# siisee11/PMDFC

Hardware: AMD Instinct MI355X
Metric: batched CCEH lookup+insert Mops/s (1/2/4/8 GPU) + % HBM random-access roofline (higher is better)
Workload: dtype u64; 1 GPU; config2: per GPU 64M unique uniform u64 keys (value=key), CCEH_hybrid(65536); 64 Insert batches of 1M then 64 Get batches of 1M (100% hit); index reset each step; the insert batches through InsertBatches (batch i+1 partitioned while batch i is applied), the Get batches through GetBatches (one launch over the 64 batches; per-op results as batch by batch); keys_per_gpu=67108864, batch=1048576, init_cap=65536, parallelism=hash-prefix shards x1

## Files before the change

pmdfc_amd/csrc/bucket.hip:

```cpp
#include <algorithm>
#include <cstdlib>
#include <cstddef>

#include "cceh_device.h"
#include "cceh_kernels.h"
#include "knobs.h"

namespace pmdfc {

constexpr int kPartThreads = 1024;
constexpr int kPartPer = (int)kPartTile / kPartThreads;

constexpr int kCW = (int)kChunkWave;
constexpr int kPer = kCW / 64;
constexpr int kBmLanes = 30;
constexpr int kRoundGuard = 64;

constexpr uint32_t kGetBit = 0x80000000u;
constexpr uint32_t kOpMask = (1u << 22) - 1;

__device__ __forceinline__ uint64_t sk_make(uint32_t seg, uint32_t op, uint32_t i, uint32_t home) {
  return ((uint64_t)seg << 39) | ((uint64_t)op << 17) | ((uint64_t)i << 8) | home;
}
__device__ __forceinline__ uint32_t sk_seg(uint64_t k) { return (uint32_t)(k >> 39); }
// ... 1314 lines not shown
      if (dmask[u] & F.unres[xc]) {
        blocked_any = true;
        continue;
      }
      const uint32_t v = F.opk[p], wo = (v & 0xFFu) * 4u, q0 = F.dst[xc];
      uint32_t occw = F.snap[p];
      bool park = false;
      for (uint32_t m = dmask[u]; m; m &= m - 1u) {
        const uint32_t rq = F.res[q0 + (uint32_t)__builtin_ctz(m)];
        const uint32_t ds = ((rq & (kSlots - 1)) - wo) & (kSlots - 1);
        park |= (rq & (kFrFull | kFrPark)) != 0;
        if ((rq & kFrClaim) && ds < kWindow) occw |= 1u << ds;
      }
      if (park) {
        nr[u] = kFrPark;
      } else if (~occw) {
        nr[u] = kFrClaim | ((wo + (uint32_t)__builtin_ctz(~occw)) & (kSlots - 1));
      } else {
        nr[u] = kFrFull;
        atomicMin(&F.bfull[xc], v >> 8);
      }
    }
    __builtin_amdgcn_wave_barrier();
#pragma unroll
    for (int u = 0; u < kLp; ++u) {
      if (!nr[u]) continue;
      const uint32_t p = (uint32_t)u * 64u + lane, xc = F.binp[p];
      F.res[p] = (uint16_t)nr[u];
      atomicAnd(&F.unres[xc], ~(1u << (p - F.dst[xc])));
      lres[u] = nr[u];
    }
    __builtin_amdgcn_wave_barrier();
    if (!__ballot(blocked_any)) break;
  }
  stamp(srow, kBsFcResolved, lane == 0);
  if (srow && lane == 0) srow[kBsFcRounds] = nrounds | ((uint64_t)ntot << 16);
}

template <bool UPS, uint32_t NL, uint32_t NB, class BinF>
__device__ __forceinline__ void fc_commit(const BucketArgs& a, uint32_t w, const FcScr<NL, NB>& F, const LaneOps& o,
                                          const bool (&pc)[kPer], const uint32_t (&st)[kPer], BinF bin,
                                          ulonglong2* wl_kv, uint32_t* wl_op, uint32_t* s_nsplit, uint32_t* s_nreq,
                                          uint32_t* s_need, WaveStat& c, const uint32_t* upd) {
  const uint32_t lbase = a.sbits + a.p1;
#pragma unroll
  for (int j = 0; j < kPer; ++j) {
    if (!o.pq[j]) continue;
    const uint32_t op = o.rop[j] & kOpMask, bf = F.bfull[bin(j)];
    const uint32_t r = st[j] & 0xFFFFu;
    const uint32_t seg = de_seg(o.e8[j]);
    if (op >= bf || (r & kFrPark)) {
      if (op == bf) {
        const uint32_t L = de_ld(o.e8[j]);
        const uint32_t ri = a.mode == 2 ? kSplitCap : atomicAdd(s_nreq, 1u);
        if (ri < kSplitCap) {
          a.req[(size_t)w * kSplitCap + ri] = make_uint2(seg | (L << 27), o.x8[j]);
          a.reqop[(size_t)w * kSplitCap + ri] = op;
          atomicMax(s_need, L + 1 - lbase);
        }
      }
      const uint32_t k = atomicAdd(s_nsplit, 1u);
      wl_kv[k] = make_ulonglong2(o.rk[j], o.rv[j]);
      wl_op[k] = o.rop[j];
      ++c.waited;
    } else if (r & kFrClaim) {
      const uint32_t sl = r & (kSlots - 1);
      a.pairs[(size_t)seg * kSlots + sl] = make_ulonglong2(o.rk[j], o.rv[j]);
      atomicOr(a.occ + (size_t)seg * 32u + (sl >> 5), 1u << (sl & 31u));
      c.lines += (((sl - o.home8[j] * 4u) & (kSlots - 1)) >> 2) + 1u;
    } else if (UPS && !pc[j]) {
      const uint32_t sl = upd[j];
      a.pairs[(size_t)seg * kSlots + sl] = make_ulonglong2(o.rk[j], o.rv[j]);
      a.st[op] = 11;
      c.lines += (((sl - o.home8[j] * 4u) & (kSlots - 1)) >> 2) + 1u;
    }
  }
}

template <uint32_t NL, uint32_t NB, bool UPS = false, class BinF>
__device__ __forceinline__ bool fast_claim(const BucketArgs& a, uint32_t w, uint32_t* sc,
                                           const uint64_t* s_key, ulonglong2* wl_kv, uint32_t* wl_op,
                                           uint32_t* s_nsplit, uint32_t* s_nreq, uint32_t* s_need,
                                           const LaneOps& o, BinF bin, WaveStat& c, uint64_t* srow,
                                           const uint32_t* upd = nullptr, const uint32_t* occw = nullptr) {
  const uint32_t lane = __lane_id() & 63u;
  const uint32_t full = a.ctl->full;
  const FcScr<NL, NB> F(sc);
  uint32_t *const hm = F.hm, *const dm = F.dm, *const cnt = F.cnt, *const dst = F.dst, *const bfull = F.bfull;
  bool pc[kPer];
#pragma unroll
  for (int j = 0; j < kPer; ++j) pc[j] = o.pq[j] && (!UPS || upd[j] == 0xFFFFu);
  uint32_t olo[kPer], ohi[kPer];
#pragma unroll
  for (int j = 0; j < kPer; ++j) {
    if (!pc[j]) continue;
    if constexpr (UPS) {
      olo[j] = occw[2 * j];
      ohi[j] = occw[2 * j + 1];
    } else {
      const uint32_t* og = a.occ + (size_t)de_seg(o.e8[j]) * 32u;
      const uint32_t wi = o.home8[j] >> 3;
      olo[j] = ld_u32_l2(og + wi);
      ohi[j] = ld_u32_l2(og + ((wi + 1u) & 31u));
    }
  }
#pragma unroll
  for (int t = 0; t < (int)(2 * NB * 8 / 64); ++t) hm[t * 64 + lane] = 0;
  if (lane < NB) {
    cnt[lane] = 0;
    bfull[lane] = 0xFFFFFFFFu;
  }
  __builtin_amdgcn_wave_barrier();
  uint32_t st[kPer];
#pragma unroll
  for (int j = 0; j < kPer; ++j)
    if (pc[j]) st[j] = atomicOr(&hm[bin(j) * 8u + (o.home8[j] >> 5)], 1u << (o.home8[j] & 31u));
#pragma unroll
  for (int j = 0; j < kPer; ++j)
    if (pc[j] && ((st[j] >> (o.home8[j] & 31u)) & 1u)) atomicOr(&dm[bin(j) * 8u + (o.home8[j] >> 5)], 1u << (o.home8[j] & 31u));
  __builtin_amdgcn_wave_barrier();
  stamp(srow, kBsBinned, lane == 0);
  if (srow && lane == 0) srow[kBsOrdered] = 0;
  constexpr uint32_t kDep = 1u << 24;
  uint64_t fk = 0;
  int fkj = -1;
#pragma unroll
  for (int j = 0; j < kPer; ++j) {
    st[j] = 0;
    if (!pc[j]) continue;
    const uint32_t h = o.home8[j], xc = bin(j), base = xc * 8u, l0 = (h - 7u) & 255u;
    const uint32_t wo = h * 4u;
    const uint32_t win = __builtin_amdgcn_alignbit(ohi[j], olo[j], wo & 31u);
    const uint32_t cl = ~win ? (uint32_t)__builtin_ctz(~win) >> 2 : 7u;
    const uint32_t w0 = hm[base + (l0 >> 5)], w1 = hm[base + (((l0 >> 5) + 1u) & 7u)];
    const uint32_t nb = __builtin_amdgcn_alignbit(w1, w0, l0 & 31u) & ((0x100u << cl) - 1u) & ~0x80u;
    const bool dup = (dm[base + (h >> 5)] >> (h & 31u)) & 1u;
    if (nb != 0 || dup) {
      const uint32_t r = atomicAdd(&cnt[xc], 1u);
      st[j] = kDep | (r << 16);
    } else if (~win) {
      st[j] = kFrClaim | ((wo + (uint32_t)__builtin_ctz(~win)) & (kSlots - 1));
    } else {
      st[j] = kFrFull;
      atomicMin(&bfull[xc], o.rop[j] & kOpMask);
      if (fkj < 0) {
        fk = ld_pair_l2(a.pairs + (size_t)de_seg(o.e8[j]) * kSlots + wo).x;
        fkj = j;
      }
    }
  }
  __builtin_amdgcn_wave_barrier();
  const uint32_t cb = lane < NB ? cnt[lane] : 0u;
  if (__ballot(cb > kDepMax)) return false;
  uint32_t ntot;
  const uint32_t ex = wave_excl_scan(cb, &ntot);
  if (lane < NB) dst[lane] = ex;
  uint32_t runs = 0;
  if (lane < NB) {
    uint32_t any = 0;
#pragma unroll
    for (int t = 0; t < 8; ++t) any |= hm[lane * 8u + t];
    runs = (uint32_t)__popcll(__ballot(any != 0));
  }
  __builtin_amdgcn_wave_barrier();
  stamp(srow, kBsBatchOrder, lane == 0);
#pragma unroll
  for (int j = 0; j < kPer; ++j) {
    if (!(st[j] & kDep)) continue;
    const uint32_t xc = bin(j), p = dst[xc] + ((st[j] >> 16) & 0xFFu);
    st[j] = kDep | (p << 16);
    F.opk[p] = ((o.rop[j] & kOpMask) << 8) | o.home8[j];
    F.snap[p] = __builtin_amdgcn_alignbit(ohi[j], olo[j], (o.home8[j] * 4u) & 31u);
    F.res[p] = 0;
    F.slot8[p] = (uint8_t)((uint32_t)j * 64u + lane);
    F.binp[p] = (uint8_t)xc;
  }
  if (lane < NB) F.unres[lane] = cb >= 32 ? 0xFFFFFFFFu : (1u << cb) - 1u;
  __builtin_amdgcn_wave_barrier();
  fc_resolve(F, ntot, srow);
#pragma unroll
  for (int j = 0; j < kPer; ++j)
    if (st[j] & kDep) st[j] |= F.res[(st[j] >> 16) & 0xFFu];
  bool fails = false;
#pragma unroll
  for (int j = 0; j < kPer; ++j) {
    if (!pc[j] || (o.rop[j] & kOpMask) != bfull[bin(j)]) continue;
    const uint32_t xc = bin(j), q0 = (st[j] & kDep) ? dst[xc] : 0u, n = (st[j] & kDep) ? cnt[xc] : 0u;
    if (fkj == j && hash64(fk) != hash64(o.rk[j])) {
      fails |= de_ld(o.e8[j]) + 1 > kMaxDepth || full;
      continue;
    }
    fails |= fc_full(a, full, o.e8[j], o.rk[j], o.home8[j] * 4u, F.res, F.slot8, s_key, q0, n) != kFrSplit;
  }
  if (__ballot(fails)) return false;
  stamp(srow, kBsRunsDone, lane == 0);
  fc_commit<UPS>(a, w, F, o, pc, st, bin, wl_kv, wl_op, s_nsplit, s_nreq, s_need, c, upd);
  if (lane == 0) c.runs += runs;
  stamp(srow, kBsWritten, lane == 0);
  return true;
}

__device__ __forceinline__ void clear_other_parity(const BucketArgs& a) {
  const uint32_t lane = __lane_id() & 63u, q = a.par ^ 1u;
  if (lane < 2 * kGShards) a.gsh[((size_t)q * kGShards + (lane % kGShards)) * kGStride + (lane / kGShards) * 16] = 0;
  if (lane == 2 * kGShards) a.ctl->nfin[q] = 0;
  if (lane == 2 * kGShards + 1) a.ctl->anyreq[q] = 0;
  if (lane == 2 * kGShards + 2) a.ctl->anydecl[q] = 0;
}


__device__ __forceinline__ void first_pass_clears(const BucketArgs& a, uint32_t w) {
  const uint32_t lane = __lane_id() & 63u;
  const uint32_t pb = w >> a.sbb, sub = w & ((1u << a.sbb) - 1);
  if (a.clear_next) {
    if (sub == 0 && lane < kPartSubs) a.cursor_next[(lane << (a.p1 - a.sbb)) + pb] = 0;
    if (w == 0 && lane == 0) *a.ovf_next = 0;
  }
  if (w == 0) clear_other_parity(a);
}

constexpr int kPre = 4;
static_assert(kPre * 64 == 32 * kPartSubs, "prefetch: 32 records per sub-region");
struct PreRecs {
  uint32_t op[kPre];
  uint64_t k[kPre], v[kPre];
};
__device__ __forceinline__ void prefetch_records(const BucketArgs& a, uint32_t pb, uint32_t half, PreRecs& pr) {
  const uint32_t lane = __lane_id() & 63u;
  const uint64_t rb0 = (uint64_t)pb * a.cap;
#pragma unroll
  for (int u = 0; u < kPre; ++u) {
    const uint32_t jj = (uint32_t)u * 64u + lane;
    const uint64_t j = rb0 + (uint64_t)(jj >> 5) * a.capx + min(half * 32u + (jj & 31u), a.capx - 1u);
    pr.op[u] = a.rop[j];
    const ulonglong2 kv = a.rkv[j];
    pr.k[u] = kv.x;
    pr.v[u] = kv.y;
  }
}
__device__ __forceinline__ bool pre_valid(const BucketArgs& a, const PreRecs& pr, int u, uint32_t half, uint32_t csub,
                                          uint32_t sub) {
  const uint32_t jj = (uint32_t)u * 64u + (__lane_id() & 63u);
  const uint32_t cs = (uint32_t)__shfl((int)csub, (int)(jj >> 5));
  return half * 32u + (jj & 31u) < cs && ((pr.op[u] >> 22) & ((1u << a.sbb) - 1)) == sub;
}
__device__ __forceinline__ uint32_t compact_prefetched(const BucketArgs& a, const PreRecs& pr, uint32_t half,
                                                       uint32_t csub, uint32_t sub, uint32_t m, ulonglong2* kv,
                                                       uint32_t* op, uint32_t cap) {
  const uint64_t lt = (1ULL << (__lane_id() & 63u)) - 1;
#pragma unroll
  for (int u = 0; u < kPre; ++u) {
    const bool match = pre_valid(a, pr, u, half, csub, sub);
    const uint64_t bal = __ballot(match);
    const uint32_t idx = m + (uint32_t)__popcll(bal & lt);
    if (match && idx < cap) {
      kv[idx] = make_ulonglong2(pr.k[u], pr.v[u]);
      op[idx] = pr.op[u];
    }
    m += (uint32_t)__popcll(bal);
  }
  return m;
}

__device__ __forceinline__ uint32_t sub_count_load(const BucketArgs& a, uint32_t pb) {
  const uint32_t lane = __lane_id() & 63u;
  return lane < kPartSubs ? min(a.cursor[(lane << (a.p1 - a.sbb)) + pb], a.capx) : 0u;
}
__device__ __forceinline__ uint32_t sub_count_max(uint32_t csub) {
  uint32_t cmax = csub;
#pragma unroll
  for (int o = 4; o > 0; o >>= 1) cmax = max(cmax, (uint32_t)__shfl_xor((int)cmax, o));
  return (uint32_t)__shfl((int)cmax, 0);
}

__device__ __forceinline__ void request_tail(const BucketArgs& a, uint32_t w, const uint32_t& nreq,
                                             const uint32_t& need, uint32_t db) {
  __builtin_amdgcn_wave_barrier();
  const uint32_t nr = min(nreq, kSplitCap);
  if (nr) request_splits(a, w, nr, need > db ? need : 0u);
}

__device__ __forceinline__ void publish_stats(const BucketArgs& a, uint32_t w, uint64_t wsv, WaveStat c) {
  const uint32_t lane = __lane_id() & 63u;
  for (int o = 32; o > 0; o >>= 1) {
    c.lines += (uint32_t)__shfl_down((int)c.lines, o);
    c.waited += (uint32_t)__shfl_down((int)c.waited, o);
  }
  const uint32_t s0 = (uint32_t)__shfl((int)c.lines, 0), s1 = (uint32_t)__shfl((int)c.waited, 0);
  const uint32_t s3 = (uint32_t)__shfl((int)c.loss, 0), s4 = (uint32_t)__shfl((int)c.runs, 0);
  const uint32_t add = lane == 0 ? s0 : lane == 1 ? s1 : lane == 2 ? c.splits : lane == 3 ? s3
                     : lane == 4 ? s4 : lane == 5 ? c.rounds : 0u;
  uint64_t* ws = a.wstat + (size_t)w * kWStat;
  if (lane < 6u && add) ws[lane] = wsv + add;
  if (lane == 3u && s3) atomicAdd(&a.ctl->loss_events, 1u);
  if (lane == 6u && (c.max_rounds || c.max_ld || c.grow)) {
    const uint64_t mr = max((uint32_t)(wsv & 0xFFFF), c.max_rounds);
    const uint64_t ml = max((uint32_t)((wsv >> 16) & 0xFF), c.max_ld);
    ws[6] = mr | (ml << 16) | (((wsv >> 32) + c.grow) << 32);
  }
  if (lane == 0 && c.bad) atomicOr(&a.ctl->err, 4u);
}



static_assert(kPre == kPer, "the prefetched records fill the chunk registers slot for slot");

struct ChunkRegs {
  uint64_t k[kPer], v[kPer];
  uint32_t op[kPer];
  bool ok[kPer];
};

struct RoundOps {
  bool pq[kPer];
  uint64_t kk[kPer];
  uint32_t ro[kPer];
  uint32_t e8[kPer], home8[kPer], x8[kPer];
};

__device__ __forceinline__ uint32_t chunk_slot(bool strided, int j) {
  const uint32_t lane = __lane_id() & 63u;
  return strided ? (uint32_t)j * 64u + lane : kPer * lane + (uint32_t)j;
}

struct LdsDir {
  bool on = false, written = false;
  uint32_t v0 = 0, v1 = 0;
};
__device__ __forceinline__ LdsDir lds_dir_load(const BucketArgs& a, uint32_t off, uint32_t db) {
  const uint32_t lane = __lane_id() & 63u;
  LdsDir d;
  d.on = (1u << db) <= kLdsDir;
  if (d.on) {
    if (lane < (1u << db)) d.v0 = ld_u32_l2(a.pool + off + lane);
    if (lane + 64u < (1u << db)) d.v1 = ld_u32_l2(a.pool + off + lane + 64u);
  }
  return d;
}

__device__ __forceinline__ void take_chunk(const ulonglong2* kv, const uint32_t* op, uint32_t m, ChunkRegs& r) {
#pragma unroll
  for (int j = 0; j < kPer; ++j) {
    const uint32_t i = (uint32_t)j * 64u + (__lane_id() & 63u);
    r.ok[j] = i < m;
    if (r.ok[j]) {
      const ulonglong2 p = kv[i];
      r.k[j] = p.x;
      r.v[j] = p.y;
      r.op[j] = op[i];
// ... 717 lines not shown
#pragma unroll
  for (int q = 0; q < kPer; ++q) {
    const uint32_t pv = q ? v[q - 1] : (lane ? prev_last : ~0u);
    const bool st = v[q] != ~0u && (pv == ~0u || (pv >> 8) != (v[q] >> 8));
    starts |= st ? 1u << q : 0u;
    s_rank[kPer * lane + q] = v[q];
  }
  uint32_t tot;
  const uint32_t rk0 = wave_excl_scan((uint32_t)__builtin_popcount(starts), &tot);
  if (lane == 0) s_sel[0] = ~0u;
  __builtin_amdgcn_wave_barrier();
  if (blockIdx.x >= tot) return;
  {
    uint32_t r = rk0;
#pragma unroll
    for (int q = 0; q < kPer; ++q)
      if ((starts >> q) & 1u) {
        if (r == blockIdx.x) {
          s_sel[0] = v[q] >> 8;
          s_sel[1] = kPer * lane + q;
        }
        ++r;
      }
  }
  __builtin_amdgcn_wave_barrier();
  const uint32_t w = s_sel[0], e0 = s_sel[1];
  uint32_t m = 0;
  for (uint32_t t0 = 0; e0 + t0 < kCW; t0 += 64) {
    const uint32_t t = t0 + lane;
    const uint32_t e = e0 + t < kCW ? s_rank[e0 + t] : ~0u;
    const bool mine = e != ~0u && (e >> 8) == w;
    const uint64_t bal = __ballot(mine);
    m += (uint32_t)__popcll(bal);
    if (mine) {
      const uint32_t i = e & 0xFFu;
      const bool ins = !ops || ops[i] == 1;
      S.kv[t] = make_ulonglong2(keys[i], ins ? vin[i] : 0ULL);
      S.op[t] = i | (ins ? 0u : kGetBit);
      if (ins && a.vout) a.vout[i] = 0;
    }
    if (bal != ~0ULL) break;
  }
  __builtin_amdgcn_wave_barrier();
  bucket_body<true, true, false>(a, w, S, m);
}

__device__ __forceinline__ bool tiny_batch(const BucketArgs& a, BucketLds<true, false>& S, uint32_t n, bool in,
                                           uint64_t key, bool ins, uint64_t val,
                                           const uint64_t* hdr_cache = nullptr) {
  const uint32_t lane = threadIdx.x & 63u;
  const uint64_t h = hash64(key);
  bool live = false;
  if (in) {
    const uint8_t bad = reserved_key(key) ? 3 : wrong_shard(h, a.sbits, a.shard) ? 8 : 0;
    if (bad) {
      a.st[lane] = bad;
      if (a.vout) a.vout[lane] = 0;
    }
    live = !bad;
  }
  const uint32_t w = live ? bucket_of(h, a.sbits, a.p1) : 0u;
  uint32_t e = 0;
  if (live) {
    const uint64_t hd = hdr_cache ? hdr_cache[w] : a.hdr[w];
    e = ld_u32_l2(a.pool + hdr_off(hd) + sub_index(h, a.sbits, a.p1, hdr_db(hd)));
  }
  const uint32_t seg = de_seg(e);
  const uint64_t lv = __ballot(live);
  bool shared = false;
  for (uint64_t m = lv; m; m &= m - 1) {
    const int j = __builtin_ctzll(m);
    const uint32_t sj = (uint32_t)__shfl((int)seg, j);
    shared |= (uint32_t)j != lane && sj == seg;
  }
  bool general = live && (shared || (ins && a.upsert));
  if (live && !general) {
    ulonglong2* sp = a.pairs + (size_t)seg * kSlots;
    if (!ins) {
      uint64_t v = 0;
      const uint8_t st = lane_probe(sp, key, h, &v);
      a.vout[lane] = v;
      a.st[lane] = st;
    } else {
      const uint32_t wi0 = (uint32_t)(h & 0xFF) * 4u, wi = wi0 >> 5, wn = (wi + 1u) & 31u;
      uint32_t* og = a.occ + (size_t)seg * 32u;
      const uint32_t lo = ld_u32_l2(og + wi), hi = ld_u32_l2(og + wn);
      const int pos = window_first_free(lo, hi, wi0);
      if (pos < 0) {
        general = true;
      } else {
        sp[pos] = make_ulonglong2(key, val);
        const uint32_t pw = (uint32_t)pos >> 5;
        og[pw] = (pw == wi ? lo : hi) | (1u << ((uint32_t)pos & 31u));
        a.st[lane] = 2;
        if (a.vout) a.vout[lane] = 0;
      }
    }
  }
  const bool any_general = __ballot(general) != 0;
  for (uint64_t gm = __ballot(general); gm;) {
    const uint32_t wb = (uint32_t)__shfl((int)w, __builtin_ctzll(gm));
    const uint64_t mine = __ballot(general && w == wb);
    if (general && w == wb) {
      const uint32_t t = (uint32_t)__popcll(mine & ((1ULL << lane) - 1));
      S.kv[t] = make_ulonglong2(key, val);
      S.op[t] = lane | (ins ? 0u : kGetBit);
      if (ins && a.vout) a.vout[lane] = 0;
    }
    __builtin_amdgcn_s_waitcnt(0);
    __builtin_amdgcn_wave_barrier();
    bucket_body<true, true, false>(a, wb, S, (uint32_t)__popcll(mine));
    __builtin_amdgcn_wave_barrier();
    gm &= ~mine;
  }
  return any_general;
}

__global__ __launch_bounds__(64, 1) void k_mixed_tiny(BucketArgs a, const uint8_t* __restrict__ ops,
                                                      const uint64_t* __restrict__ keys,
                                                      const uint64_t* __restrict__ vin) {
  __shared__ BucketLds<true, false> S;
  const uint32_t lane = threadIdx.x, n = (uint32_t)a.n;
  const bool in = lane < n;
  const uint64_t key = in ? keys[lane] : kInvalid;
  const bool ins = in && (!ops || ops[lane] == 1);
  const uint64_t val = ins ? vin[lane] : 0ULL;
  tiny_batch(a, S, n, in, key, ins, val);
}

__device__ __forceinline__ uint32_t sys_ld32(const uint32_t* p) {
  return __hip_atomic_load(p, __ATOMIC_RELAXED, __HIP_MEMORY_SCOPE_SYSTEM);
}
__device__ __forceinline__ uint64_t sys_ld64(const uint64_t* p) {
  return __hip_atomic_load(p, __ATOMIC_RELAXED, __HIP_MEMORY_SCOPE_SYSTEM);
}
__device__ __forceinline__ void sys_st32(uint32_t* p, uint32_t v) {
  __hip_atomic_store(p, v, __ATOMIC_RELAXED, __HIP_MEMORY_SCOPE_SYSTEM);
}
__device__ __forceinline__ void sys_st64(uint64_t* p, uint64_t v) {
  __hip_atomic_store(p, v, __ATOMIC_RELAXED, __HIP_MEMORY_SCOPE_SYSTEM);
}

__global__ __launch_bounds__(64, 1) void k_serve(ServeArgs sa) {
  __shared__ BucketLds<true, false> S;
  const uint32_t lane = threadIdx.x;
  const uint64_t mask = sa.ring_size - 1;
  if (sa.nwaves > 1) {
    sa.req += (size_t)blockIdx.x * sa.ring_size;
    sa.resp += (size_t)blockIdx.x * sa.ring_size;
    sa.ctl += blockIdx.x;
    sa.head0 = sys_ld64(&sa.ctl->head);
  }
  uint64_t head = sa.head0, chunks = 0, reloads = 0;
  uint64_t hb = sys_ld64(&sa.ctl->heartbeat);
  uint64_t t_hb = (uint64_t)wall_clock64(), t_last = t_hb;
  bool idle_set = false;
  uint64_t tp[5] = {0, 0, 0, 0, 0};
  const uint64_t t_start = t_hb;
  const auto put_prof = [&] {
    const uint64_t life = (uint64_t)wall_clock64() - t_start;
    if (lane < 6)
      sys_st64(&sa.ctl->prof[lane],
               lane == 0 ? tp[0] : lane == 1 ? tp[1] : lane == 2 ? tp[2] : lane == 3 ? tp[3] : lane == 4 ? tp[4] : life);
    if (lane == 6) sys_st64(&sa.ctl->head, head);
    if (lane == 7) sys_st64(&sa.ctl->chunks, chunks);
    if (lane == 8) sys_st64(&sa.ctl->reloads, reloads);
  };
  __shared__ uint8_t s_st[64];
  __shared__ uint64_t s_vout[64];
// ... 146 lines not shown
      if (!ok) a.ctl->full = 1;
    }
    if (!ok) {
      if (gs + nr <= a.max_segments && (!team || wv == 0)) {
        retire_segment(a.pairs, a.occ, a.ldep, seg0 + k);
        if (lane == 0) atomicAdd(&a.ctl->dead, 1u);
      }
      continue;
    }
    bool b = false;
    uint64_t* stp = a.stamps && k < kSplitStamps ? a.stamps + (size_t)k * 8 : nullptr;
    stamp(stp, kSsStart, lane == 0 && (!team || wv == 0));
    const uint32_t trig = a.drops ? a.reqop[(size_t)w * kSplitCap + i] : 0u;
    const uint32_t ps = el.x & ((1u << 27) - 1), pl = el.x >> 27;
    if (team) {
      loss += split_team<4>(a.pairs, a.occ, a.ldep, ps, seg0 + k, pl, &s_scr[0][0], &b, stp, a.drops, &a.ctl->drop_n,
                            trig, wv);
    } else {
      uint32_t so = wv * kSplitScratch;
      __asm__ volatile("" : "+v"(so));
      loss += wave_split(a.pairs, a.occ, a.ldep, ps, seg0 + k, pl, &s_scr[0][0] + so, &b, stp, a.drops,
                         &a.ctl->drop_n, trig);
    }
    bad |= b;
  }
  if (lane == 0 && (!team || wv == 0)) {
    if (loss) {
      atomicAdd(reinterpret_cast<unsigned long long*>(&a.ctl->split_loss), (unsigned long long)loss);
      atomicAdd(&a.ctl->loss_events, 1u);
    }
    if (bad) atomicOr(&a.ctl->err, 4u);
  }
}

static SplitArgs split_args(const BucketArgs& a, uint64_t* stamps, uint32_t team_max) {
  SplitArgs p;
  p.par = a.par;
  p.pfix = a.pfix;
  p.stamps = stamps;
  p.gsh = a.gsh;
  p.gsplit = a.gsplit;
  p.gcap = a.gcap;
  p.act = a.act;
  p.gbase = a.gbase;
  p.ngrant = a.ngrant;
  p.newoff = a.newoff;
  p.need = a.need;
  p.max_segments = a.max_segments;
  p.pool_cap = a.pool_cap;
  p.pairs = a.pairs;
  p.occ = a.occ;
  p.ldep = a.ldep;
  p.ctl = a.ctl;
  p.reqop = a.reqop;
  p.drops = a.drops;
  p.team_max = team_max;
  return p;
}

template <bool WIDE>
struct FastCfg {
  static constexpr int FP = WIDE ? 2 : 3;
  static constexpr uint32_t FC = 64u * (uint32_t)FP;
  static constexpr uint32_t NB = WIDE ? 64u : kFastBins;
  static constexpr uint32_t MaxDb = WIDE ? 7u : 5u;
};

template <bool WIDE>
struct FastLds {
  using C = FastCfg<WIDE>;
  union {
    uint32_t sc[FcLayout<C::FC, C::NB>::Words];
    struct {
      ulonglong2 kv[C::FC];
      uint32_t op[C::FC];
    } stage;
  };
  uint32_t seen[4];
  uint32_t nsplit, nreq, need;
};

constexpr uint32_t kCpWaves = 1u << kCpSbb;
constexpr uint32_t kCpPre = 192;
struct CpLds {
  union {
    FastLds<false> w[kCpWaves];
    struct {
      ulonglong2 kv[kPartSubs * kCpPre];
      uint32_t op[kPartSubs * kCpPre];
      uint16_t idx[kCpWaves][FastCfg<false>::FC];
    } st;
  };
  uint32_t csub[kPartSubs];
};
static_assert(sizeof(CpLds) <= 40 * 1024, "4 workgroups of 8 waves per CU");

__device__ __forceinline__ bool dense_bins(uint32_t* seen, const bool (&pq)[kPer], uint32_t (&bn)[kPer], uint32_t nb) {
  __builtin_amdgcn_wave_barrier();
#pragma unroll
  for (int j = 0; j < kPer; ++j)
    if (pq[j]) atomicOr(&seen[bn[j] >> 5], 1u << (bn[j] & 31u));
  __builtin_amdgcn_wave_barrier();
  const uint32_t s0 = seen[0], s1 = seen[1], s2 = seen[2], s3 = seen[3];
  if (__builtin_popcount(s0) + __builtin_popcount(s1) + __builtin_popcount(s2) + __builtin_popcount(s3) > (int)nb)
    return false;
#pragma unroll
  for (int j = 0; j < kPer; ++j) {
    const uint32_t x = bn[j], q = x >> 5, below = (1u << (x & 31u)) - 1u;
    uint32_t r = __builtin_popcount((q == 0 ? s0 : q == 1 ? s1 : q == 2 ? s2 : s3) & below);
    r += q > 0 ? __builtin_popcount(s0) : 0;
    r += q > 1 ? __builtin_popcount(s1) : 0;
    r += q > 2 ? __builtin_popcount(s2) : 0;
    bn[j] = r;
  }
  return true;
}

__device__ __forceinline__ bool upsert_probe(const BucketArgs& a, const bool (&pq)[kPer], const uint64_t (&rk)[kPer],
                                             const uint32_t (&e8)[kPer], const uint32_t (&home8)[kPer],
                                             uint32_t (&upd)[kPer], uint32_t (&occw)[2 * kPer]) {
  const uint32_t lane = __lane_id() & 63u;
  uint32_t hv[4];
#pragma unroll
  for (int q = 0; q < 4; ++q) hv[q] = q < kPer && pq[q] ? (uint32_t)hash64(rk[q]) : 0xFFFFFFFFu;
  wave_sort32<4>(hv, 256);
  bool dup = false;
#pragma unroll
  for (int q = 0; q < 3; ++q) dup |= hv[q] != 0xFFFFFFFFu && hv[q] == hv[q + 1];
  const uint32_t nx = (uint32_t)__shfl_down((int)hv[0], 1);
  dup |= lane < 63u && hv[3] != 0xFFFFFFFFu && hv[3] == nx;
  if (__ballot(dup)) return false;
  uint32_t nl[kPer];
#pragma unroll
  for (int j = 0; j < kPer; ++j) {
    upd[j] = 0xFFFFu;
    occw[2 * j] = occw[2 * j + 1] = 0;
    if (!pq[j]) continue;
    const uint32_t* og = a.occ + (size_t)de_seg(e8[j]) * 32u;
    const uint32_t wi = home8[j] >> 3;
    occw[2 * j] = ld_u32_l2(og + wi);
    occw[2 * j + 1] = ld_u32_l2(og + ((wi + 1u) & 31u));
  }
#pragma unroll
  for (int j = 0; j < kPer; ++j) {
    const uint32_t win = __builtin_amdgcn_alignbit(occw[2 * j + 1], occw[2 * j], (home8[j] * 4u) & 31u);
    const uint32_t ff = ~win ? (uint32_t)__builtin_ctz(~win) : 32u;
    nl[j] = pq[j] ? (ff + 3u) >> 2 : 0u;
  }
  for (uint32_t t = 0;; ++t) {
    bool more = false;
#pragma unroll
    for (int j = 0; j < kPer; ++j) more |= t < nl[j] && upd[j] == 0xFFFFu;
    if (!__ballot(more)) break;
    uint64_t kq[kPer][4];
#pragma unroll
    for (int j = 0; j < kPer; ++j) {
      if (t >= nl[j] || upd[j] != 0xFFFFu) continue;
      const ulonglong2* ln = a.pairs + (size_t)de_seg(e8[j]) * kSlots + ((home8[j] + t) & 255u) * 4u;
#pragma unroll
      for (int q = 0; q < 4; ++q) kq[j][q] = reinterpret_cast<const uint64_t*>(ln + q)[0];
    }
#pragma unroll
    for (int j = 0; j < kPer; ++j) {
      if (t >= nl[j] || upd[j] != 0xFFFFu) continue;
#pragma unroll
      for (int q = 3; q >= 0; --q)
        if (kq[j][q] == rk[j]) upd[j] = ((home8[j] + t) * 4u + (uint32_t)q) & (kSlots - 1);
    }
  }
  return true;
}

template <bool WIDE, bool UPS = false, bool CP = false>
__device__ __forceinline__ uint32_t apply_fast(const BucketArgs& a, FastLds<WIDE>& S, uint32_t w,
                                               CpLds* cpl = nullptr) {
  using C = FastCfg<WIDE>;
  static_assert(!CP || (!WIDE && !UPS), "the coarse-partition pass is the lean insert-only one");
  const uint32_t lane = threadIdx.x & 63u;
  const uint32_t pb = w >> a.sbb, sub = w & ((1u << a.sbb) - 1);
  uint64_t* const srow = bucket_stamp_row(a, w);
  stamp(srow, kBsStart, lane == 0);
  first_pass_clears(a, w);
  PreRecs pr;
  constexpr int kCpLd = (int)(kPartSubs * kCpPre / (64 * kCpWaves));
  static_assert(kCpLd <= kPre, "the staging loads use the prefetch registers");
  if constexpr (CP) {
    const uint64_t rb0 = (uint64_t)pb * a.cap;
#pragma unroll
    for (int u = 0; u < kCpLd; ++u) {
      const uint32_t t = (uint32_t)u * 64u * kCpWaves + threadIdx.x;
      const uint64_t j = rb0 + (uint64_t)(t / kCpPre) * a.capx + min(t % kCpPre, a.capx - 1u);
      pr.op[u] = a.rop[j];
      const ulonglong2 kv = a.rkv[j];
      pr.k[u] = kv.x;
      pr.v[u] = kv.y;
    }
  } else {
    prefetch_records(a, pb, 0, pr);
  }
  const uint32_t csub = sub_count_load(a, pb);
  const uint64_t wsv = lane < 7u ? a.wstat[(size_t)w * kWStat + lane] : 0ULL;
  const uint32_t* fslot = a.pool + (size_t)w * kFixedSlot;
  const uint32_t spec0 = (a.pfix && (WIDE || lane < 32u)) ? ld_u32_l2(fslot + lane) : 0u;
  const uint32_t spec1 = (WIDE && a.pfix) ? ld_u32_l2(fslot + 64u + lane) : 0u;
  const uint64_t hd = a.hdr[w];
  const uint32_t off = hdr_off(hd), db = hdr_db(hd);
  const uint32_t novf = *a.ovf;
  const bool fixed = a.pfix && off == w * kFixedSlot && db <= kFixedBits;
  uint32_t dv0, dv1 = 0u;
  if (fixed) {
    dv0 = lane < (1u << db) ? spec0 : 0u;
    dv1 = lane + 64u < (1u << db) ? spec1 : 0u;
  } else {
    dv0 = (db <= C::MaxDb && lane < (1u << db)) ? ld_u32_l2(a.pool + off + lane) : 0u;
    if (WIDE) dv1 = (db <= C::MaxDb && lane + 64u < (1u << db)) ? ld_u32_l2(a.pool + off + 64u + lane) : 0u;
  }
  const uint32_t cmax = sub_count_max(csub);
  bool pq[kPer];
  uint64_t rk[kPer], rv[kPer];
  uint32_t rop[kPer];
  if constexpr (CP) {
#pragma unroll
    for (int u = 0; u < kCpLd; ++u) {
      const uint32_t t = (uint32_t)u * 64u * kCpWaves + threadIdx.x;
      cpl->st.op[t] = pr.op[u];
      cpl->st.kv[t] = make_ulonglong2(pr.k[u], pr.v[u]);
    }
    __syncthreads();
    uint32_t dec = (db > C::MaxDb || novf != 0) ? 2u : cmax > kCpPre ? 2u : 0u;
    uint32_t m = 0;
    if (!dec) {
      const uint64_t lt = (1ULL << lane) - 1;
      const uint32_t v = w & (kCpWaves - 1);
      uint16_t* my = cpl->st.idx[v];
#pragma unroll 4
      for (uint32_t c = 0; c < kPartSubs * kCpPre / 64; ++c) {
        const uint32_t t = c * 64u + lane;
        const uint32_t cs = (uint32_t)__shfl((int)csub, (int)(t / kCpPre));
        const uint32_t r = cpl->st.op[t];
        const bool match = t % kCpPre < cs && ((r >> 22) & (kCpWaves - 1)) == v;
        const uint64_t bal = __ballot(match);
        const uint32_t idx = m + (uint32_t)__popcll(bal & lt);
        if (match && idx < C::FC) my[idx] = (uint16_t)t;
        m += (uint32_t)__popcll(bal);
      }
      if (m > C::FC) dec = 1u;
      __builtin_amdgcn_wave_barrier();
#pragma unroll
      for (int j = 0; j < kPer; ++j) {
        const uint32_t i = (uint32_t)j * 64u + lane;
        pq[j] = !dec && j < C::FP && i < m;
        rk[j] = rv[j] = 0;
        rop[j] = 0;
        if (pq[j]) {
          const uint32_t t = my[i];
          const ulonglong2 kv = cpl->st.kv[t];
          rk[j] = kv.x;
          rv[j] = kv.y;
          rop[j] = cpl->st.op[t];
        }
      }
    }
    __syncthreads();
    if (dec) return dec;
  } else {
    if (db > C::MaxDb || novf != 0) return 2u;
    if (cmax > C::FC) return 1u;
    uint32_t m = 0;
    for (uint32_t half = 0; half * 32u < cmax; ++half) {
      if (half) prefetch_records(a, pb, half, pr);
      m = compact_prefetched(a, pr, half, csub, sub, m, S.stage.kv, S.stage.op, C::FC);
    }
    if (m > C::FC) return 1u;
    __builtin_amdgcn_wave_barrier();
#pragma unroll
    for (int j = 0; j < kPer; ++j) {
      const uint32_t i = (uint32_t)j * 64u + lane;
      pq[j] = j < C::FP && i < m;
      rk[j] = rv[j] = 0;
      rop[j] = 0;
      if (pq[j]) {
        const ulonglong2 kv = S.stage.kv[i];
        rk[j] = kv.x;
        rv[j] = kv.y;
        rop[j] = S.stage.op[i];
      }
    }
    __builtin_amdgcn_wave_barrier();
  }
  if (lane == 0) {
    S.nsplit = 0;
    S.nreq = 0;
    S.need = db;
  }
  if (WIDE && lane < 4) S.seen[lane] = 0;
  uint32_t e8[kPer], home8[kPer], x8[kPer], bn[WIDE ? kPer : 1];
  (void)bn;
#pragma unroll
  for (int j = 0; j < kPer; ++j) {
    home8[j] = x8[j] = 0;
    if (pq[j]) {
      const uint64_t h = hash64(rk[j]);
      home8[j] = (uint32_t)(h & 0xFF);
      x8[j] = sub_index(h, a.sbits, a.p1, db);
    }
    const uint32_t lo = (uint32_t)__shfl((int)dv0, (int)(x8[j] & 63u));
    if (WIDE) {
      const uint32_t hi = (uint32_t)__shfl((int)dv1, (int)(x8[j] & 63u));
      e8[j] = x8[j] < 64u ? lo : hi;
    } else {
      e8[j] = lo;
    }
  }
  const auto first_sub = [&](int j) -> uint32_t { return first_sub_index(a, db, x8[j], e8[j]); };
  if constexpr (WIDE) {
#pragma unroll
    for (int j = 0; j < kPer; ++j) bn[j] = pq[j] ? first_sub(j) : 0u;
    if (!dense_bins(S.seen, pq, bn, C::NB)) return 1u;
  }
  uint32_t upd[UPS ? kPer : 1], occw[UPS ? 2 * kPer : 1];
  if constexpr (UPS) {
    if (!upsert_probe(a, pq, rk, e8, home8, upd, occw)) return 1u;
  }
  stamp(srow, kBsLoaded, lane == 0);
  WaveStat c;
  const auto bin = [&](int j) -> uint32_t {
    if constexpr (WIDE) return bn[j];
    else return first_sub(j);
  };
  if (!fast_claim<C::FC, C::NB, UPS>(a, w, S.sc, nullptr, a.wl_kv + (size_t)w * kCW, a.wl_op + (size_t)w * kCW,
                                     &S.nsplit, &S.nreq, &S.need, LaneOps{rk, rv, rop, pq, e8, home8, x8}, bin, c, srow,
                                     UPS ? upd : nullptr, UPS ? occw : nullptr))
    return 1u;
  if (lane == 0) a.wl_n[w] = S.nsplit;
  request_tail(a, w, S.nreq, S.need, db);
  c.rounds = c.max_rounds = 1;
  publish_stats(a, w, wsv, c);
  stamp(srow, kBsEnd, lane == 0);
  return 0u;
}

__device__ __forceinline__ void declined(const BucketArgs& a, uint32_t w) {
  a.fbl[w] |= 1u;
  a.ctl->anydecl[a.par] = 1u;
}

__global__ __launch_bounds__(64, 8) void k_apply_fast(BucketArgs a) {
  if (gated_off(a)) return;
  __shared__ FastLds<false> S;
  if (apply_fast<false>(a, S, blockIdx.x) != 0 && threadIdx.x == 0) declined(a, blockIdx.x);
}

#ifndef PMDFC_CP_WPE
#define PMDFC_CP_WPE 8
#endif
__global__ __launch_bounds__(64 * kCpWaves) __attribute__((amdgpu_waves_per_eu(PMDFC_CP_WPE, 8))) void k_apply_fast_cp(
    BucketArgs a) {
  if (gated_off(a)) return;
  __shared__ CpLds L;
  const uint32_t v = (uint32_t)__builtin_amdgcn_readfirstlane((int)(threadIdx.x >> 6)), w = (blockIdx.x << kCpSbb) | v;
  if (apply_fast<false, false, true>(a, L.w[v], w, &L) != 0 && (threadIdx.x & 63u) == 0) declined(a, w);
}

__global__ __launch_bounds__(64, 6) void k_apply_wide(BucketArgs a) {
  if (gated_off(a)) return;
  __shared__ FastLds<true> S;
  if (apply_fast<true>(a, S, blockIdx.x) != 0 && threadIdx.x == 0) declined(a, blockIdx.x);
}

template <bool WIDE>
__global__ __launch_bounds__(64, 5) void k_apply_fast_ups(BucketArgs a) {
  __shared__ FastLds<WIDE> S;
  if (apply_fast<WIDE, true>(a, S, blockIdx.x) != 0 && threadIdx.x == 0) declined(a, blockIdx.x);
}

__global__ __launch_bounds__(64, 2) void k_apply_fb(BucketArgs a) {
  if (gated_off(a)) return;
  const uint32_t w = blockIdx.x, f = a.fbl[w];
  if (!(f & 1u)) return;
  __shared__ BucketLds<false, true> S;
  bucket_body<false, false, true>(a, w, S);
  if (threadIdx.x == 0) a.fbl[w] = f + 1u;
}


#ifndef PMDFC_PARKED_GRID
#define PMDFC_PARKED_GRID 3072
#endif
#ifndef PMDFC_FINAL_GRID
#define PMDFC_FINAL_GRID 256
#endif
constexpr uint32_t kParkedGrid = PMDFC_PARKED_GRID;
constexpr uint32_t kFinalGrid = PMDFC_FINAL_GRID;
#ifndef PMDFC_MIXED_SMALL_GRID
#define PMDFC_MIXED_SMALL_GRID 256
#endif
constexpr uint32_t kMixedSmallGrid = PMDFC_MIXED_SMALL_GRID;
#ifndef PMDFC_PARKED_GRID_RAMP
#define PMDFC_PARKED_GRID_RAMP 4096
#endif
#ifndef PMDFC_FINAL_GRID_RAMP
#define PMDFC_FINAL_GRID_RAMP 1024
#endif
constexpr uint32_t kParkedGridRamp = PMDFC_PARKED_GRID_RAMP;
constexpr uint32_t kFinalGridRamp = PMDFC_FINAL_GRID_RAMP;

uint32_t part_blocks(uint64_t n) { return (uint32_t)((n + kPartTile - 1) / kPartTile); }

void launch_part(const PartArgs& a, hipStream_t s) {
  if (!a.n) return;
  hipLaunchKernelGGL(k_part, dim3(part_blocks(a.n)), dim3(kPartThreads), 0, s, a);
}

void launch_apply(const BucketLaunch& L, uint32_t mode, hipStream_t s) {
  if (!L.a.n) return;
// ... 89 lines not shown
```

pmdfc_amd/csrc/cceh_device.h:

```cpp
#pragma once
#include <hip/hip_runtime.h>
#include <stdint.h>

namespace pmdfc {

constexpr uint32_t kSlots = 1024;
constexpr uint32_t kWindow = 32;
constexpr uint32_t kLines = 8;
constexpr uint32_t kMaxDepth = 30;
constexpr uint64_t kInvalid = ~0ULL;
constexpr uint64_t kSentinel = ~0ULL - 1;
constexpr uint8_t kStPending = 0xFF;
constexpr uint8_t kStLinked = 0xFE;
constexpr uint8_t kStJoin = 0xFD;
constexpr uint32_t kJoinReps = 8;
constexpr uint32_t kJoinBits = 1u << 20;
constexpr uint64_t kJoinWords = (uint64_t)kJoinBits / 32 * kJoinReps;
__host__ __device__ __forceinline__ uint64_t iset_slot(uint64_t h, uint64_t mask) {
  return (h ^ (h >> 29) ^ (h >> 47)) & mask;
}

__host__ __device__ __forceinline__ uint64_t hash64(uint64_t key) {
  const uint64_t mul = 0xc6a4a7935bd1e995ULL;
  uint64_t h = 0xc70697ULL ^ (8ULL * mul);
// ... 7 lines not shown

__host__ __device__ __forceinline__ uint32_t murmur2_u64(uint64_t key, uint32_t seed) {
  const uint32_t m = 0x5bd1e995u;
  uint32_t h = seed ^ 8u;
  uint32_t k = (uint32_t)key;
  k *= m; k ^= k >> 24; k *= m;
  h *= m; h ^= k;
  k = (uint32_t)(key >> 32);
  k *= m; k ^= k >> 24; k *= m;
  h *= m; h ^= k;
  h ^= h >> 13; h *= m; h ^= h >> 15;
  return h;
}

__host__ __device__ __forceinline__ uint64_t splitmix64(uint64_t x) {
  uint64_t z = x + 0x9E3779B97F4A7C15ULL;
  z = (z ^ (z >> 30)) * 0xBF58476D1CE4E5B9ULL;
  z = (z ^ (z >> 27)) * 0x94D049BB133111EBULL;
  return z ^ (z >> 31);
}

__host__ __device__ __forceinline__ bool reserved_key(uint64_t k) {
  return k >= kSentinel;
}

constexpr uint32_t kSegBits = 26;
constexpr uint32_t kSegMask = (1u << kSegBits) - 1;
constexpr uint64_t kMaxSegments = 1ULL << 25;
__host__ __device__ __forceinline__ uint32_t de_seg(uint32_t e) { return e & kSegMask; }
__host__ __device__ __forceinline__ uint32_t de_ld(uint32_t e) { return e >> kSegBits; }
__host__ __device__ __forceinline__ uint32_t de_make(uint32_t seg, uint32_t ld) {
  return seg | (ld << kSegBits);
}

struct Geo {
  const uint64_t* hdr;
  const uint32_t* pool;
  uint32_t p1;
  uint32_t sbits;
  uint32_t shard;
  const uint32_t* flat;
  const uint32_t* flat_bits;
};
constexpr uint32_t kFlatMaxBits = 20;

__host__ __device__ __forceinline__ uint32_t hdr_off(uint64_t hd) { return (uint32_t)hd; }
__host__ __device__ __forceinline__ uint32_t hdr_db(uint64_t hd) { return (uint32_t)(hd >> 32) & 0xFFu; }
__host__ __device__ __forceinline__ uint64_t hdr_make(uint32_t off, uint32_t db) {
  return (uint64_t)off | ((uint64_t)db << 32);
}

__device__ __forceinline__ uint32_t bucket_of(uint64_t h, uint32_t sbits, uint32_t p1) {
  return p1 ? (uint32_t)((h << sbits) >> (64 - p1)) : 0u;
}
__device__ __forceinline__ uint32_t sub_index(uint64_t h, uint32_t sbits, uint32_t p1, uint32_t db) {
  return db ? (uint32_t)((h << (sbits + p1)) >> (64 - db)) : 0u;
}

__device__ __forceinline__ uint32_t dir_entry(const Geo& g, uint64_t h) {
  if (g.flat) {
    const uint32_t fb = *g.flat_bits;
    if (fb <= kFlatMaxBits) return g.flat[fb ? (uint32_t)((h << g.sbits) >> (64 - fb)) : 0u];
  }
  const uint64_t hd = g.hdr[bucket_of(h, g.sbits, g.p1)];
  return g.pool[hdr_off(hd) + sub_index(h, g.sbits, g.p1, hdr_db(hd))];
}

__device__ __forceinline__ bool wrong_shard(uint64_t h, uint32_t sbits, uint32_t shard) {
  return sbits != 0 && (uint32_t)(h >> (64 - sbits)) != shard;
}

typedef unsigned long long u64x2_t __attribute__((ext_vector_type(2)));
typedef unsigned int u32x4_t __attribute__((ext_vector_type(4)));
__device__ __forceinline__ ulonglong2 ld_pair_l2(const ulonglong2* p) {
  const u64x2_t v = __builtin_nontemporal_load(reinterpret_cast<const u64x2_t*>(p));
  return make_ulonglong2(v.x, v.y);
}
__device__ __forceinline__ uint4 ld_u4_l2(const uint32_t* p) {
  const u32x4_t v = __builtin_nontemporal_load(reinterpret_cast<const u32x4_t*>(p));
  return make_uint4(v.x, v.y, v.z, v.w);
}
__device__ __forceinline__ uint32_t ld_u32_l2(const uint32_t* p) {
  return __hip_atomic_load(p, __ATOMIC_RELAXED, __HIP_MEMORY_SCOPE_AGENT);
}

__device__ __forceinline__ int window_first_free(uint32_t lo, uint32_t hi, uint32_t w) {
  uint64_t win = (((uint64_t)hi << 32) | lo) >> (w & 31);
  uint32_t fr = ~(uint32_t)win;
  if (fr == 0) return -1;
  return (int)((w + (uint32_t)__builtin_ctz(fr)) & (kSlots - 1));
}

__device__ __forceinline__ uint64_t shfl64(uint64_t v, int src) {
  int lo = __shfl((int)(uint32_t)v, src);
  int hi = __shfl((int)(uint32_t)(v >> 32), src);
  return ((uint64_t)(uint32_t)hi << 32) | (uint32_t)lo;
}

__device__ __forceinline__ uint8_t quad_probe(const ulonglong2* __restrict__ seg, uint64_t key,
                                              uint64_t h, uint32_t q, uint64_t* val,
                                              uint32_t* lines) {
  const uint32_t line0 = (uint32_t)(h & 0xFF);
  const uint32_t qbase = (__lane_id() & 63u) & ~3u;
  for (uint32_t t = 0; t < kLines;) {
    const uint32_t ln = (line0 + t) & 255u;
    const bool two = !(ln & 1u) && t + 1 < kLines;
    const ulonglong2 pa = seg[ln * 4u + q];
    const ulonglong2 pb = two ? seg[ln * 4u + 4u + q] : pa;
#pragma unroll
    for (uint32_t k = 0; k < 2; ++k) {
      if (k == 1 && !two) break;
      const ulonglong2 p = k ? pb : pa;
      const uint32_t mn = (uint32_t)(__ballot(p.x == key) >> qbase) & 0xFu;
      const uint32_t en = (uint32_t)(__ballot(p.x == kInvalid) >> qbase) & 0xFu;
      if (mn) {
        *val = shfl64(p.y, (int)(qbase + (uint32_t)__builtin_ctz(mn)));
        *lines = t + k + 1;
        return 1;
      }
      if (en) {
        *lines = t + k + 1;
        return 0;
      }
    }
    t += two ? 2u : 1u;
  }
  *lines = kLines;
  return 0;
}

__device__ __forceinline__ uint8_t quad_probe_once(const ulonglong2* __restrict__ seg, uint64_t key,
                                                   uint64_t h, uint32_t q, uint64_t* val) {
  const uint32_t line0 = (uint32_t)(h & 0xFF);
  const uint32_t qbase = (__lane_id() & 63u) & ~3u;
  uint32_t copies = 0;
  for (uint32_t t = 0; t < kLines;) {
    const uint32_t ln = (line0 + t) & 255u;
    const bool two = !(ln & 1u) && t + 1 < kLines;
    const ulonglong2 pa = seg[ln * 4u + q];
    const ulonglong2 pb = two ? seg[ln * 4u + 4u + q] : pa;
    bool stop = false;
#pragma unroll
    for (uint32_t k = 0; k < 2; ++k) {
      if (k == 1 && !two) break;
      const ulonglong2 p = k ? pb : pa;
      const uint32_t mn = (uint32_t)(__ballot(p.x == key) >> qbase) & 0xFu;
      const uint32_t en = (uint32_t)(__ballot(p.x == kInvalid) >> qbase) & 0xFu;
      if (mn && copies == 0) *val = shfl64(p.y, (int)(qbase + (uint32_t)__builtin_ctz(mn)));
      copies += (uint32_t)__builtin_popcount(mn);
      if (en || copies > 1) {
        stop = true;
        break;
      }
    }
    if (stop) break;
    t += two ? 2u : 1u;
  }
  return copies == 0 ? 0 : copies == 1 ? 1 : 2;
}

__device__ __forceinline__ uint8_t lane_probe(const ulonglong2* __restrict__ seg, uint64_t key,
                                              uint64_t h, uint64_t* val) {
  const uint32_t line0 = (uint32_t)(h & 0xFF);
  for (uint32_t t = 0; t < kLines; t += 2) {
    ulonglong2 ln[8];
#pragma unroll
// ... 139 lines not shown
```

Measured before the change: 13520 Mops/s.

## Split compaction staging loads into lean first stage and gated second stage

Refactors occupancy-window loads behind a WinLd helper. An optional 64-bit atomic load is added but left off by default. In the CP compaction path, the staging loads are split into a 128-record first stage and a 64-record second stage. The second stage is skipped when a sub-region's count does not reach it, and the header, overflow and count loads are issued early so they overlap the record loads. The compaction scan now walks each sub-region only up to its count, which is meant to avoid useless loads and LDS reads in exchange for more complex indexing and extra readlane work.

```diff
diff --git a/pmdfc_amd/csrc/bucket.hip b/pmdfc_amd/csrc/bucket.hip
--- a/pmdfc_amd/csrc/bucket.hip
+++ b/pmdfc_amd/csrc/bucket.hip
@@ -1420,7 +1420,7 @@
                                            const uint64_t* s_key, ulonglong2* wl_kv, uint32_t* wl_op,
                                            uint32_t* s_nsplit, uint32_t* s_nreq, uint32_t* s_need,
                                            const LaneOps& o, BinF bin, WaveStat& c, uint64_t* srow,
-                                           const uint32_t* upd = nullptr, const uint32_t* occw = nullptr) {
+                                           const uint32_t* upd = nullptr, const uint32_t* owin = nullptr) {
   const uint32_t lane = __lane_id() & 63u;
   const uint32_t full = a.ctl->full;
   const FcScr<NL, NB> F(sc);
@@ -1428,20 +1428,16 @@
   bool pc[kPer];
 #pragma unroll
   for (int j = 0; j < kPer; ++j) pc[j] = o.pq[j] && (!UPS || upd[j] == 0xFFFFu);
-  uint32_t olo[kPer], ohi[kPer];
-#pragma unroll
-  for (int j = 0; j < kPer; ++j) {
-    if (!pc[j]) continue;
-    if constexpr (UPS) {
-      olo[j] = occw[2 * j];
-      ohi[j] = occw[2 * j + 1];
-    } else {
-      const uint32_t* og = a.occ + (size_t)de_seg(o.e8[j]) * 32u;
-      const uint32_t wi = o.home8[j] >> 3;
-      olo[j] = ld_u32_l2(og + wi);
-      ohi[j] = ld_u32_l2(og + ((wi + 1u) & 31u));
-    }
-  }
+  WinLd ow[UPS ? 1 : kPer];
+  if constexpr (!UPS) {
+#pragma unroll
+    for (int j = 0; j < kPer; ++j)
+      if (pc[j]) ow[j] = ld_window_l2(a.occ + (size_t)de_seg(o.e8[j]) * 32u, o.home8[j] >> 3);
+  }
+  const auto wbits = [&](int j) -> uint32_t {
+    if constexpr (UPS) return owin[j];
+    else return window_bits(ow[j], o.home8[j]);
+  };
 #pragma unroll
   for (int t = 0; t < (int)(2 * NB * 8 / 64); ++t) hm[t * 64 + lane] = 0;
   if (lane < NB) {
@@ -1468,7 +1464,7 @@
     if (!pc[j]) continue;
     const uint32_t h = o.home8[j], xc = bin(j), base = xc * 8u, l0 = (h - 7u) & 255u;
     const uint32_t wo = h * 4u;
-    const uint32_t win = __builtin_amdgcn_alignbit(ohi[j], olo[j], wo & 31u);
+    const uint32_t win = wbits(j);
     const uint32_t cl = ~win ? (uint32_t)__builtin_ctz(~win) >> 2 : 7u;
     const uint32_t w0 = hm[base + (l0 >> 5)], w1 = hm[base + (((l0 >> 5) + 1u) & 7u)];
     const uint32_t nb = __builtin_amdgcn_alignbit(w1, w0, l0 & 31u) & ((0x100u << cl) - 1u) & ~0x80u;
@@ -1508,7 +1504,7 @@
     const uint32_t xc = bin(j), p = dst[xc] + ((st[j] >> 16) & 0xFFu);
     st[j] = kDep | (p << 16);
     F.opk[p] = ((o.rop[j] & kOpMask) << 8) | o.home8[j];
-    F.snap[p] = __builtin_amdgcn_alignbit(ohi[j], olo[j], (o.home8[j] * 4u) & 31u);
+    F.snap[p] = wbits(j);
     F.res[p] = 0;
     F.slot8[p] = (uint8_t)((uint32_t)j * 64u + lane);
     F.binp[p] = (uint8_t)xc;
@@ -1600,9 +1596,12 @@
   return m;
 }
 
+__device__ __forceinline__ uint32_t sub_count_issue(const BucketArgs& a, uint32_t pb) {
+  const uint32_t lane = __lane_id() & 63u;
+  return a.cursor[((lane % kPartSubs) << (a.p1 - a.sbb)) + pb];
+}
 __device__ __forceinline__ uint32_t sub_count_load(const BucketArgs& a, uint32_t pb) {
-  const uint32_t lane = __lane_id() & 63u;
-  return lane < kPartSubs ? min(a.cursor[(lane << (a.p1 - a.sbb)) + pb], a.capx) : 0u;
+  return min(sub_count_issue(a, pb), a.capx);
 }
 __device__ __forceinline__ uint32_t sub_count_max(uint32_t csub) {
   uint32_t cmax = csub;
@@ -2486,9 +2485,10 @@
       a.vout[lane] = v;
       a.st[lane] = st;
     } else {
-      const uint32_t wi0 = (uint32_t)(h & 0xFF) * 4u, wi = wi0 >> 5, wn = (wi + 1u) & 31u;
+      const uint32_t wi0 = (uint32_t)(h & 0xFF) * 4u, wi = wi0 >> 5;
       uint32_t* og = a.occ + (size_t)seg * 32u;
-      const uint32_t lo = ld_u32_l2(og + wi), hi = ld_u32_l2(og + wn);
+      const uint2 ow = window_words(ld_window_l2(og, wi), wi);
+      const uint32_t lo = ow.x, hi = ow.y;
       const int pos = window_first_free(lo, hi, wi0);
       if (pos < 0) {
         general = true;
@@ -2801,6 +2801,10 @@
 
 constexpr uint32_t kCpWaves = 1u << kCpSbb;
 constexpr uint32_t kCpPre = 192;
+#ifndef PMDFC_CP_LEAN_STAGE
+#define PMDFC_CP_LEAN_STAGE 1
+#endif
+constexpr uint32_t kCpPre1 = PMDFC_CP_LEAN_STAGE ? 128 : kCpPre;
 struct CpLds {
   union {
     FastLds<false> w[kCpWaves];
@@ -2837,7 +2841,7 @@
 
 __device__ __forceinline__ bool upsert_probe(const BucketArgs& a, const bool (&pq)[kPer], const uint64_t (&rk)[kPer],
                                              const uint32_t (&e8)[kPer], const uint32_t (&home8)[kPer],
-                                             uint32_t (&upd)[kPer], uint32_t (&occw)[2 * kPer]) {
+                                             uint32_t (&upd)[kPer], uint32_t (&owin)[kPer]) {
   const uint32_t lane = __lane_id() & 63u;
   uint32_t hv[4];
 #pragma unroll
@@ -2850,19 +2854,16 @@
   dup |= lane < 63u && hv[3] != 0xFFFFFFFFu && hv[3] == nx;
   if (__ballot(dup)) return false;
   uint32_t nl[kPer];
+  WinLd ow[kPer];
 #pragma unroll
   for (int j = 0; j < kPer; ++j) {
     upd[j] = 0xFFFFu;
-    occw[2 * j] = occw[2 * j + 1] = 0;
-    if (!pq[j]) continue;
-    const uint32_t* og = a.occ + (size_t)de_seg(e8[j]) * 32u;
-    const uint32_t wi = home8[j] >> 3;
-    occw[2 * j] = ld_u32_l2(og + wi);
-    occw[2 * j + 1] = ld_u32_l2(og + ((wi + 1u) & 31u));
+    ow[j] = WinLd{};
+    if (pq[j]) ow[j] = ld_window_l2(a.occ + (size_t)de_seg(e8[j]) * 32u, home8[j] >> 3);
   }
 #pragma unroll
   for (int j = 0; j < kPer; ++j) {
-    const uint32_t win = __builtin_amdgcn_alignbit(occw[2 * j + 1], occw[2 * j], (home8[j] * 4u) & 31u);
+    const uint32_t win = owin[j] = window_bits(ow[j], home8[j]);
     const uint32_t ff = ~win ? (uint32_t)__builtin_ctz(~win) : 32u;
     nl[j] = pq[j] ? (ff + 3u) >> 2 : 0u;
   }
@@ -2902,29 +2903,53 @@
   first_pass_clears(a, w);
   PreRecs pr;
   constexpr int kCpLd = (int)(kPartSubs * kCpPre / (64 * kCpWaves));
+  constexpr int kCpLd1 = (int)(kPartSubs * kCpPre1 / (64 * kCpWaves));
   static_assert(kCpLd <= kPre, "the staging loads use the prefetch registers");
-  if constexpr (CP) {
-    const uint64_t rb0 = (uint64_t)pb * a.cap;
-#pragma unroll
-    for (int u = 0; u < kCpLd; ++u) {
-      const uint32_t t = (uint32_t)u * 64u * kCpWaves + threadIdx.x;
-      const uint64_t j = rb0 + (uint64_t)(t / kCpPre) * a.capx + min(t % kCpPre, a.capx - 1u);
-      pr.op[u] = a.rop[j];
-      const ulonglong2 kv = a.rkv[j];
-      pr.k[u] = kv.x;
-      pr.v[u] = kv.y;
-    }
-  } else {
-    prefetch_records(a, pb, 0, pr);
-  }
-  const uint32_t csub = sub_count_load(a, pb);
+  static_assert(kCpLd1 * 64 * kCpWaves == kPartSubs * kCpPre1 && (kCpLd - kCpLd1) * 64 * kCpWaves == kPartSubs * (kCpPre - kCpPre1),
+                "whole loads per stage");
+  const auto cp_slot = [&](int u) -> uint32_t {
+    const uint32_t t = (uint32_t)u * 64u * kCpWaves + threadIdx.x;
+    if (u < kCpLd1) return (t / kCpPre1) * kCpPre + t % kCpPre1;
+    const uint32_t r = t - kPartSubs * kCpPre1;
+    return (r / (kCpPre - kCpPre1)) * kCpPre + kCpPre1 + r % (kCpPre - kCpPre1);
+  };
+  const auto cp_load = [&](int u) {
+    const uint32_t s = cp_slot(u);
+    const uint64_t j = (uint64_t)pb * a.cap + (uint64_t)(s / kCpPre) * a.capx + min(s % kCpPre, a.capx - 1u);
+    pr.op[u] = a.rop[j];
+    const ulonglong2 kv = a.rkv[j];
+    pr.k[u] = kv.x;
+    pr.v[u] = kv.y;
+  };
   const uint64_t wsv = lane < 7u ? a.wstat[(size_t)w * kWStat + lane] : 0ULL;
   const uint32_t* fslot = a.pool + (size_t)w * kFixedSlot;
   const uint32_t spec0 = (a.pfix && (WIDE || lane < 32u)) ? ld_u32_l2(fslot + lane) : 0u;
   const uint32_t spec1 = (WIDE && a.pfix) ? ld_u32_l2(fslot + 64u + lane) : 0u;
-  const uint64_t hd = a.hdr[w];
+  uint64_t hd = a.hdr[w];
+  uint32_t novf = *a.ovf;
+  uint32_t craw = sub_count_issue(a, pb);
+  if constexpr (CP) {
+#pragma unroll
+    for (int u = 0; u < kCpLd1; ++u) cp_load(u);
+    asm volatile("" : "+v"(craw));
+  } else {
+    prefetch_records(a, pb, 0, pr);
+  }
+  const uint32_t csub = min(craw, a.capx);
+  bool live2 = false;
+  if constexpr (CP && kCpLd1 < kCpLd) {
+    static_assert(kCpLd - kCpLd1 == 1 && kCpPre - kCpPre1 == 64, "wave v loads the second stage of sub-region v");
+    const uint32_t cv = (uint32_t)__builtin_amdgcn_readlane((int)csub, (int)(w & (kCpWaves - 1)));
+    live2 = kCpPre1 + lane < cv;
+    if (live2) cp_load(kCpLd1);
+  }
+  if constexpr (CP) {
+    uint32_t hl = (uint32_t)hd, hh = (uint32_t)(hd >> 32);
+    asm volatile("" : "+v"(hl), "+v"(hh), "+v"(novf));
+    hd = (uint64_t)(uint32_t)__builtin_amdgcn_readfirstlane((int)hh) << 32 | (uint32_t)__builtin_amdgcn_readfirstlane((int)hl);
+    novf = (uint32_t)__builtin_amdgcn_readfirstlane((int)novf);
+  }
   const uint32_t off = hdr_off(hd), db = hdr_db(hd);
-  const uint32_t novf = *a.ovf;
   const bool fixed = a.pfix && off == w * kFixedSlot && db <= kFixedBits;
   uint32_t dv0, dv1 = 0u;
   if (fixed) {
@@ -2941,7 +2966,8 @@
   if constexpr (CP) {
 #pragma unroll
     for (int u = 0; u < kCpLd; ++u) {
-      const uint32_t t = (uint32_t)u * 64u * kCpWaves + threadIdx.x;
+      if (u >= kCpLd1 && !live2) continue;
+      const uint32_t t = cp_slot(u);
       cpl->st.op[t] = pr.op[u];
       cpl->st.kv[t] = make_ulonglong2(pr.k[u], pr.v[u]);
     }
@@ -2952,16 +2978,24 @@
       const uint64_t lt = (1ULL << lane) - 1;
       const uint32_t v = w & (kCpWaves - 1);
       uint16_t* my = cpl->st.idx[v];
-#pragma unroll 4
-      for (uint32_t c = 0; c < kPartSubs * kCpPre / 64; ++c) {
-        const uint32_t t = c * 64u + lane;
-        const uint32_t cs = (uint32_t)__shfl((int)csub, (int)(t / kCpPre));
-        const uint32_t r = cpl->st.op[t];
-        const bool match = t % kCpPre < cs && ((r >> 22) & (kCpWaves - 1)) == v;
-        const uint64_t bal = __ballot(match);
-        const uint32_t idx = m + (uint32_t)__popcll(bal & lt);
-        if (match && idx < C::FC) my[idx] = (uint16_t)t;
-        m += (uint32_t)__popcll(bal);
+      for (uint32_t xs = 0; xs < kPartSubs; ++xs) {
+        const uint32_t cs = (uint32_t)__builtin_amdgcn_readlane((int)csub, (int)xs);
+        uint32_t r[kCpPre / 64];
+#pragma unroll
+        for (uint32_t q = 0; q < kCpPre / 64; ++q) {
+          const uint32_t i = q * 64u + lane;
+          r[q] = i < cs ? cpl->st.op[xs * kCpPre + i] : ~0u;
+        }
+#pragma unroll
+        for (uint32_t q = 0; q < kCpPre / 64; ++q) {
+          if (q * 64u >= cs) break;
+          const uint32_t i = q * 64u + lane;
+          const bool match = i < cs && ((r[q] >> 22) & (kCpWaves - 1)) == v;
+          const uint64_t bal = __ballot(match);
+          const uint32_t idx = m + (uint32_t)__popcll(bal & lt);
+          if (match && idx < C::FC) my[idx] = (uint16_t)(xs * kCpPre + i);
+          m += (uint32_t)__popcll(bal);
+        }
       }
       if (m > C::FC) dec = 1u;
       __builtin_amdgcn_wave_barrier();
@@ -3037,9 +3071,9 @@
     for (int j = 0; j < kPer; ++j) bn[j] = pq[j] ? first_sub(j) : 0u;
     if (!dense_bins(S.seen, pq, bn, C::NB)) return 1u;
   }
-  uint32_t upd[UPS ? kPer : 1], occw[UPS ? 2 * kPer : 1];
+  uint32_t upd[UPS ? kPer : 1], owin[UPS ? kPer : 1];
   if constexpr (UPS) {
-    if (!upsert_probe(a, pq, rk, e8, home8, upd, occw)) return 1u;
+    if (!upsert_probe(a, pq, rk, e8, home8, upd, owin)) return 1u;
   }
   stamp(srow, kBsLoaded, lane == 0);
   WaveStat c;
@@ -3049,7 +3083,7 @@
   };
   if (!fast_claim<C::FC, C::NB, UPS>(a, w, S.sc, nullptr, a.wl_kv + (size_t)w * kCW, a.wl_op + (size_t)w * kCW,
                                      &S.nsplit, &S.nreq, &S.need, LaneOps{rk, rv, rop, pq, e8, home8, x8}, bin, c, srow,
-                                     UPS ? upd : nullptr, UPS ? occw : nullptr))
+                                     UPS ? upd : nullptr, UPS ? owin : nullptr))
     return 1u;
   if (lane == 0) a.wl_n[w] = S.nsplit;
   request_tail(a, w, S.nreq, S.need, db);
diff --git a/pmdfc_amd/csrc/cceh_device.h b/pmdfc_amd/csrc/cceh_device.h
--- a/pmdfc_amd/csrc/cceh_device.h
+++ b/pmdfc_amd/csrc/cceh_device.h
@@ -113,6 +113,24 @@
 }
 __device__ __forceinline__ uint32_t ld_u32_l2(const uint32_t* p) {
   return __hip_atomic_load(p, __ATOMIC_RELAXED, __HIP_MEMORY_SCOPE_AGENT);
+}
+#ifndef PMDFC_OCC_X2
+#define PMDFC_OCC_X2 0
+#endif
+struct WinLd {
+  uint64_t v;
+};
+__device__ __forceinline__ WinLd ld_window_l2(const uint32_t* row, uint32_t wi) {
+  if (PMDFC_OCC_X2 && wi < 31u)
+    return {__hip_atomic_load(reinterpret_cast<const uint64_t*>(row + wi), __ATOMIC_RELAXED, __HIP_MEMORY_SCOPE_AGENT)};
+  return {ld_u32_l2(row + wi) | (uint64_t)ld_u32_l2(row + ((wi + 1u) & 31u)) << 32};
+}
+__device__ __forceinline__ uint2 window_words(const WinLd& r, uint32_t) {
+  return make_uint2((uint32_t)r.v, (uint32_t)(r.v >> 32));
+}
+__device__ __forceinline__ uint32_t window_bits(const WinLd& r, uint32_t line) {
+  const uint2 w = window_words(r, line >> 3);
+  return __builtin_amdgcn_alignbit(w.y, w.x, (line * 4u) & 31u);
 }
 
 __device__ __forceinline__ int window_first_free(uint32_t lo, uint32_t hi, uint32_t w) {
```

Measured after the change: 13750 Mops/s (median of 6 runs). 1.7% higher.
